# paramhanji/sin-inn

Measured on AMD Instinct MI355X. Metric: training frames/sec at 256x256 bs=16, higher is better.
Workload: dtype f32; 1 GPU; BASELINE configs[1]: 8-block INN (SRF, -c 4 x 2 levels), 256x256x3, fp32, synthetic clip (64 frames, lr_window 10), batch 16/GPU, full training step (fwd+bwd, rev+bwd, Adam); height=256, width=256, global_batch=16, num_coupling=4, architecture=SRF, parallelism=dp1, hip_graph=False

## Files before the change

### sin-inn_amd/csrc/conv_mfma.hip

```cpp
#include "conv_mfma_impl.h"

namespace sininn {

int conv_dispatch_k3(ConvDev& d, hipStream_t st, int force_cfg);
int conv_dispatch_k1(ConvDev& d, hipStream_t st, int force_cfg);
int conv32_dispatch_k3(ConvDev& d, hipStream_t st, int force_cfg, bool must);
int conv32_dispatch_k1(ConvDev& d, hipStream_t st, int force_cfg, bool must);
int wino_dispatch_k3(ConvDev& d, hipStream_t st, int cg2);

int g_conv_dma = 0;
static int g_force_cfg = 0;
static int g_force_ck = 0;
static int g_ablate = 0;

int conv_bf16_launch(const sininn_conv_args* a, hipStream_t st);
extern int g_bf16_force_ck16;

int conv_prepare(const sininn_conv_args* a, ConvDev& d) {
  SININN_CHECK(a != nullptr, "conv: null args");
  SININN_CHECK(a->ksize == 1 || a->ksize == 3, "conv: ksize %d not in {1,3}", a->ksize);
  SININN_CHECK(a->Cin > 0 && a->Cin % 8 == 0, "conv: Cin=%d must be a positive multiple of 8", a->Cin);
  SININN_CHECK(a->Np > 0 && a->Np % 16 == 0, "conv: Np=%d must be a positive multiple of 16", a->Np);
  SININN_CHECK(a->B > 0 && a->H > 0 && a->W > 0, "conv: bad image shape %dx%dx%d", a->B, a->H, a->W);
  SININN_CHECK((long)a->B * a->H * a->W * (long)(a->in_stride > a->out_stride ? a->in_stride : a->out_stride) < (1l << 31),
               "conv: tensor too large for 32-bit pixel offsets");
  SININN_CHECK(a->in && a->w && a->out, "conv: null tensor pointer");
  SININN_CHECK((a->in_stride >= a->Cin || a->in_group_stride > 0) && a->in_stride % 4 == 0 && aligned16(a->in),
               "conv: input must be 16-byte aligned with stride %% 4 == 0 (stride=%d)", a->in_stride);
  SININN_CHECK(aligned16(a->w), "conv: packed weights must be 16-byte aligned");
  const bool couple = a->mode == SININN_CONV_COUPLE_FWD || a->mode == SININN_CONV_COUPLE_INV;
  if (couple) {
    SININN_CHECK(a->Co > 0 && a->Co % 8 == 0 && a->Np == 2 * a->Co, "conv: coupling needs Np == 2*Co, Co %% 8 == 0 (Np=%d Co=%d)", a->Np, a->Co);
    SININN_CHECK(a->v != nullptr && a->v_stride >= a->Co, "conv: coupling needs v");
    SININN_CHECK(a->clamp > 0.f, "conv: clamp must be > 0");
    SININN_CHECK(a->out_stride >= a->Co, "conv: out_stride < Co");
  } else {
    SININN_CHECK(a->N > 0 && a->N <= a->Np && (a->out_stride >= a->N || a->out_group_stride > 0), "conv: bad N=%d (Np=%d, out_stride=%d)", a->N, a->Np, a->out_stride);
    if (a->mode == SININN_CONV_RELU) SININN_CHECK(a->bias != nullptr, "conv: RELU mode needs bias");
    if (a->mode == SININN_CONV_MASK) SININN_CHECK(a->mask != nullptr && (a->mask_stride >= a->N || a->mask_group_stride > 0), "conv: MASK mode needs mask");
    const bool cbwd = a->mode == SININN_CONV_ADD_CBWD_FWD || a->mode == SININN_CONV_ADD_CBWD_INV;
    if (a->mode == SININN_CONV_ADD || cbwd) SININN_CHECK(a->addend != nullptr, "conv: ADD mode needs addend");
    if (cbwd) SININN_CHECK(a->v && a->sbuf && a->out2 && a->Co == a->N && a->out_stride >= 2 * a->Co && a->clamp > 0.f, "conv: ADD_CBWD needs v, sbuf, out2, Co == N, out_stride >= 2*Co");
    if ((a->mode == SININN_CONV_LINEAR || a->mode == SININN_CONV_ADD) && a->mask)
      SININN_CHECK(a->Co >= 0 && a->Co % 4 == 0 && a->mask_stride >= a->N && a->mask_stride % 4 == 0 && aligned16(a->mask) && a->mask_group_stride <= 0,
                   "conv: LeakyReLU tail needs Co %% 4 == 0 and a 16-byte aligned pixel-major mask (Co=%d, mask_stride=%d)", a->Co, a->mask_stride);
    if (a->mode == SININN_CONV_IRN_FWD || a->mode == SININN_CONV_IRN_INV)
      SININN_CHECK(a->mask && a->v && a->mask_stride >= a->N && a->v_stride >= a->N && a->clamp > 0.f, "conv: IRN modes need aux (mask), v and clamp");
  }
  SININN_CHECK(aligned16(a->out) && a->out_stride % 4 == 0, "conv: out must be 16-byte aligned with stride %% 4 == 0");
  SININN_CHECK(!a->bias || aligned16(a->bias), "conv: bias must be 16-byte aligned");
  if (couple) {
    SININN_CHECK(aligned16(a->v) && a->v_stride % 4 == 0, "conv: v must be 16-byte aligned with stride %% 4 == 0");
    SININN_CHECK(!a->out2 || (aligned16(a->out2) && a->out2_stride % 4 == 0), "conv: out2 must be 16-byte aligned");
    SININN_CHECK(!a->sbuf || aligned16(a->sbuf), "conv: sbuf must be 16-byte aligned");
  }
  if (a->mode == SININN_CONV_MASK) SININN_CHECK(aligned16(a->mask) && a->mask_stride % 4 == 0, "conv: mask must be 16-byte aligned");
  SININN_CHECK(a->N % 4 == 0 || couple, "conv: N must be a multiple of 4");
  if ((a->mode == SININN_CONV_ADD || a->mode == SININN_CONV_ADD_CBWD_FWD || a->mode == SININN_CONV_ADD_CBWD_INV) && !a->addend_map)
    SININN_CHECK(aligned16(a->addend) && a->addend_stride % 4 == 0, "conv: addend must be 16-byte aligned");
  d.in = a->in; d.in_stride = a->in_stride; d.Cin = a->Cin;
  d.w = a->w; d.bias = a->bias; d.Np = a->Np;
  d.B = a->B; d.H = a->H; d.W = a->W;
  d.out = a->out; d.out_stride = a->out_stride; d.N = a->N; d.out_map = a->out_map;
  d.v = a->v; d.v_stride = a->v_stride; d.out2 = a->out2; d.out2_stride = a->out2_stride;
  d.sbuf = a->sbuf; d.logdet = a->logdet; d.Co = a->Co; d.clamp = a->clamp;
  d.mask = a->mask; d.mask_stride = a->mask_stride;
  d.addend = a->addend; d.addend_stride = a->addend_stride; d.addend_map = a->addend_map;
  d.mode = a->mode;
  d.col_tile = a->col_tile;
  d.stamp = a->stamp;
  d.ablate = g_ablate;
  d.in_chunk = a->in_group_stride > 0 ? a->in_group_stride : 8;
  d.out_gs = a->out_group_stride > 0 ? (size_t)a->out_group_stride : 0;
  d.mask_gs = a->mask_group_stride > 0 ? (size_t)a->mask_group_stride : 0;
  if (d.out_gs || d.mask_gs) {
    SININN_CHECK(a->winograd && (a->mode == SININN_CONV_RELU || a->mode == SININN_CONV_MASK) && a->N % 64 == 0 && a->N == a->Np,
                 "conv: channel-group-major out / mask needs a Winograd RELU / MASK conv with N == Np, N %% 64 == 0");
    SININN_CHECK(!d.mask_gs || a->mode == SININN_CONV_MASK, "conv: mask_group_stride without MASK mode");
  }
  if (a->in_group_stride > 0) SININN_CHECK(a->winograd && a->in_stride == 8, "conv: the channel-group-major input layout needs the Winograd kernels and in_stride == 8");
  if (a->winograd) {
    SININN_CHECK((unsigned long long)a->H * a->W * a->in_stride * 4ull < (1ull << 31),
                 "conv: one image of the input (%d x %d x stride %d floats) exceeds the 2 GB a Winograd block addresses", a->H, a->W, a->in_stride);
    SININN_CHECK((unsigned long long)(a->Cin / 8) * (unsigned long long)d.in_chunk * 4ull < (1ull << 32), "conv: input channel-group stride too large");
  }
  SININN_CHECK(a->mode >= 0 && a->mode <= SININN_CONV_ADD_CBWD_INV, "conv: unknown mode %d", a->mode);
  int ck = 8;
  for (int c : {32, 24, 16, 8}) if (a->Cin % c == 0) { ck = c; break; }
  if (g_force_ck && a->Cin % g_force_ck == 0 && g_force_ck % 8 == 0 && g_force_ck <= 32) ck = g_force_ck;
  d.CK = ck;
  d.tiles_x = d.tiles_y = 0;
  return 0;
}

int conv_launch(const sininn_conv_args* a, hipStream_t st) {
  SININN_CHECK(a != nullptr, "conv: null args");
  if (a->w_bf16) return conv_bf16_launch(a, st);
  ConvDev d;
  if (int rc = conv_prepare(a, d)) return rc;
  const bool couple = a->mode == SININN_CONV_COUPLE_FWD || a->mode == SININN_CONV_COUPLE_INV;
  if (a->winograd) {
    SININN_CHECK(a->ksize == 3, "conv: the Winograd pack needs ksize 3");
    d.col_tile = (couple && a->col_tile == 32) ? 32 : 16;
    if (couple && d.col_tile == 32) SININN_CHECK(a->Co % 16 == 0, "conv: col_tile 32 needs Co %% 16 == 0");
    return wino_dispatch_k3(d, st, g_force_cfg % 16);
  }
  const int tile = couple ? (a->col_tile == 32 ? 32 : 16) : ((a->Np % 32 == 0 && g_force_cfg < 10) ? 32 : 16);
  if (couple && tile == 32) SININN_CHECK(a->Co % 16 == 0, "conv: col_tile 32 needs Co %% 16 == 0 (Co=%d)", a->Co);
  const int fc = g_force_cfg % 10;
  if (tile == 32) {
    const int rc = (a->ksize == 3) ? conv32_dispatch_k3(d, st, fc, couple) : conv32_dispatch_k1(d, st, fc, couple);
    if (rc >= 0) return rc;
  }
  if (a->ksize == 3) return conv_dispatch_k3(d, st, fc);
  return conv_dispatch_k1(d, st, fc);
}

void conv_set_test_hooks(int force_cfg, int force_ck) {
  g_force_cfg = force_cfg % 100; g_force_ck = force_ck; g_ablate = force_cfg / 1000;
  g_bf16_force_ck16 = force_ck == 16;
  const int dma = (force_cfg / 100) % 10;
  if (dma) g_conv_dma = (dma == 1);
}

}
```

### sin-inn_amd/csrc/wino_impl.h

```cpp
#pragma once
#include "conv_mfma_impl.h"
#include "wino32_impl.h"

namespace sininn {

template <int NT, int HT, int CG>
__global__ __launch_bounds__(256 * CG, 2 / CG) void wino_kernel(ConvDev p) {
  constexpr int CK = 8;
  constexpr int NTHR = 256 * CG;
  constexpr int IW = 18, NPIX_IN = 18 * 18;
  constexpr int BG = NT * 16;
  constexpr int BN = CG * BG;
  constexpr int SI = 12, SU = 12;
  constexpr int PITCH = IW * SI + 4;
  constexpr int IN_F4 = (NPIX_IN * 2 + NTHR - 1) / NTHR;
  constexpr int U_F4 = (16 * BN * 2 + NTHR - 1) / NTHR;
  constexpr int IN_BUF = IW * PITCH + 4, U_BUF = 16 * BN * SU;
  constexpr bool U_EXACT = (16 * BN * 2) % NTHR == 0;

  extern __shared__ __attribute__((aligned(16))) float smem[];
  float* const in_lds0 = smem;
  float* const in_lds1 = smem + IN_BUF;
  float* const u_lds0 = smem + 2 * IN_BUF;
  float* const u_lds1 = u_lds0 + U_BUF;

  const int tid = threadIdx.x;
  stamp_begin(p);
  const int wave = (tid >> 6) & 3, grp = tid >> 8, lane = tid & 63;
  const int li = lane & 15, kq = lane >> 4;

  int bid = blockIdx.x;
  const int tx = bid % p.tiles_x; bid /= p.tiles_x;
  const int ty = bid % p.tiles_y;
  const int b = bid / p.tiles_y;
  const int y0 = ty * 16, x0 = tx * 16;
  const int n0 = blockIdx.y * BN;

  unsigned in_goff[IN_F4]; int in_loff[IN_F4];
#pragma unroll
  for (int r = 0; r < IN_F4; ++r) {
    const int f = tid + NTHR * r;
    const int pix = f >> 1, c4 = f & 1;
    const int py = pix / IW, px = pix - py * IW;
    const int gy = y0 + py - 1, gx = x0 + px - 1;
    const bool inside = pix < NPIX_IN;
    const bool inimg = inside && gy >= 0 && gy < p.H && gx >= 0 && gx < p.W;
    in_loff[r] = inside ? (py * PITCH + ((py >> 1) & 1) * 4 + px * SI + c4 * 4) : IW * PITCH;
    in_goff[r] = inimg ? (unsigned)(((gy * p.W + gx) * p.in_stride + c4 * 4) * 4) : BUF_OOB;
  }
  unsigned u_goff[U_F4]; int u_loff[U_F4];
#pragma unroll
  for (int r = 0; r < U_F4; ++r) {
    const int f = tid + NTHR * r;
    const int c4 = f & 1, col = (f >> 1) % BN, pos = (f >> 1) / BN;
    const bool inside = pos < 16;
    u_loff[r] = (U_EXACT || inside) ? ((pos * BN + col) * SU + c4 * 4) : -1;
    u_goff[r] = (inside && (n0 + col) < p.Np) ? (unsigned)(((pos * (p.Cin / CK) * p.Np + n0 + col) * CK + c4 * 4) * 4) : BUF_OOB;
  }
  const int nchunks = p.Cin / CK;

  const __amdgpu_buffer_rsrc_t in_rs = buf_rsrc(p.in + (size_t)b * p.H * p.W * p.in_stride), u_rs = buf_rsrc(p.w);
  const unsigned in_step = (unsigned)p.in_chunk * 4u, u_step = (unsigned)(p.Np * CK) * 4u;
  f32x4 in_reg[IN_F4], u_reg[U_F4];
  auto load_chunk = [&](int chunk) {
#pragma unroll
    for (int r = 0; r < IN_F4; ++r) in_reg[r] = buf_load4(in_rs, in_goff[r], (unsigned)chunk * in_step);
#pragma unroll
    for (int r = 0; r < U_F4; ++r) u_reg[r] = buf_load4(u_rs, u_goff[r], (unsigned)chunk * u_step);
  };
  auto store_chunk = [&](float* idst, float* udst) {
#pragma unroll
    for (int r = 0; r < IN_F4; ++r)
      *reinterpret_cast<f32x4*>(idst + in_loff[r]) = in_reg[r];
#pragma unroll
    for (int r = 0; r < U_F4; ++r)
      if (U_EXACT || u_loff[r] >= 0) *reinterpret_cast<f32x4*>(udst + u_loff[r]) = u_reg[r];
  };

  const int a_ty = 2 * wave + (li >> 3), a_tx = li & 7;
  const int a_base01 = (2 * a_ty) * PITCH + (a_ty & 1) * 4 + (2 * a_tx) * SI + 2 * kq;
  const int a_base23 = (2 * a_ty) * PITCH + ((a_ty + 1) & 1) * 4 + (2 * a_tx) * SI + 2 * kq;
  const int b_base = (grp * BG + li) * SU + 2 * kq;

  f32x4 acc[16][NT];
#pragma unroll
  for (int q = 0; q < 16; ++q)
#pragma unroll
    for (int n = 0; n < NT; ++n) acc[q][n] = (f32x4){0.f, 0.f, 0.f, 0.f};
  const bool tile1_live = (n0 + grp * BG + 16) < p.Np;

  load_chunk(0);
  store_chunk(in_lds0, u_lds0);
  if (nchunks > 1) load_chunk(1);
  __syncthreads();

  for (int it = 0; it < nchunks; ++it) {
    if (!(p.ablate & 1)) {
      if (it + 1 < nchunks) store_chunk(((it + 1) & 1) ? in_lds1 : in_lds0, ((it + 1) & 1) ? u_lds1 : u_lds0);
      if (it + 2 < nchunks) load_chunk(it + 2);
    }
    const unsigned A01 = lds_addr(((it & 1) ? in_lds1 : in_lds0) + a_base01);
    const unsigned A23 = lds_addr(((it & 1) ? in_lds1 : in_lds0) + a_base23);
    const unsigned Uc = lds_addr(((it & 1) ? u_lds1 : u_lds0) + b_base);

    f32x2 v[4][4];
    {
      f32x2 d[4][4];
      static_for<0, 16>([&](auto i) {
        constexpr int a = decltype(i)::value >> 2, c = decltype(i)::value & 3;
        d[a][c] = lds_read_b64<(a * PITCH + c * SI) * 4>(a < 2 ? A01 : A23);
      });
      asm volatile("s_waitcnt lgkmcnt(0)"
                   : "+v"(d[0][0]), "+v"(d[0][1]), "+v"(d[0][2]), "+v"(d[0][3]), "+v"(d[1][0]), "+v"(d[1][1]), "+v"(d[1][2]),
                     "+v"(d[1][3]), "+v"(d[2][0]), "+v"(d[2][1]), "+v"(d[2][2]), "+v"(d[2][3]), "+v"(d[3][0]), "+v"(d[3][1]),
                     "+v"(d[3][2]), "+v"(d[3][3]));
      f32x2 t[4][4];
#pragma unroll
      for (int c = 0; c < 4; ++c) {
        t[0][c] = d[0][c] - d[2][c];
        t[1][c] = d[1][c] + d[2][c];
        t[2][c] = d[2][c] - d[1][c];
        t[3][c] = d[1][c] - d[3][c];
      }
#pragma unroll
      for (int a = 0; a < 4; ++a) {
        v[a][0] = t[a][0] - t[a][2];
        v[a][1] = t[a][1] + t[a][2];
        v[a][2] = t[a][2] - t[a][1];
        v[a][3] = t[a][1] - t[a][3];
      }
    }
    constexpr int PF = 2;
    static_assert(NT == 2, "the wait counts below assume two column tiles per wave");
    f32x2 bf[PF + 1][NT];
    auto positions = [&](auto live1_tag) {
      constexpr bool LIVE1 = decltype(live1_tag)::value;
      static_for<0, PF>([&](auto qq) {
        constexpr int q = decltype(qq)::value;
        bf[q][0] = lds_read_b64<((q * BN) * SU) * 4>(Uc);
        if constexpr (LIVE1) bf[q][1] = lds_read_b64<((q * BN + 16) * SU) * 4>(Uc);
      });
      static_for<0, 16>([&](auto qq) {
        constexpr int q = decltype(qq)::value;
        if constexpr (q + PF < 16) {
          bf[(q + PF) % (PF + 1)][0] = lds_read_b64<(((q + PF) * BN) * SU) * 4>(Uc);
          if constexpr (LIVE1) bf[(q + PF) % (PF + 1)][1] = lds_read_b64<(((q + PF) * BN + 16) * SU) * 4>(Uc);
        }
        constexpr int newer = (q + PF < 16 ? PF : 15 - q) * (LIVE1 ? 2 : 1);
        if constexpr (LIVE1) lds_wait<newer>(bf[q % (PF + 1)][0], bf[q % (PF + 1)][1]);
        else lds_wait<newer>(bf[q % (PF + 1)][0]);
        acc[q][0] = __builtin_amdgcn_mfma_f32_16x16x4f32(v[q >> 2][q & 3].x, bf[q % (PF + 1)][0].x, acc[q][0], 0, 0, 0);
        if constexpr (LIVE1) acc[q][1] = __builtin_amdgcn_mfma_f32_16x16x4f32(v[q >> 2][q & 3].x, bf[q % (PF + 1)][1].x, acc[q][1], 0, 0, 0);
        acc[q][0] = __builtin_amdgcn_mfma_f32_16x16x4f32(v[q >> 2][q & 3].y, bf[q % (PF + 1)][0].y, acc[q][0], 0, 0, 0);
        if constexpr (LIVE1) acc[q][1] = __builtin_amdgcn_mfma_f32_16x16x4f32(v[q >> 2][q & 3].y, bf[q % (PF + 1)][1].y, acc[q][1], 0, 0, 0);
      });
    };
    if (tile1_live) positions(std::true_type{}); else positions(std::false_type{});
    if (!(p.ablate & 2)) __syncthreads();
  }

  {
    constexpr int TS = BN + 4;
    float* const T = smem;
#pragma unroll
    for (int n = 0; n < NT; ++n)
#pragma unroll
      for (int r = 0; r < 4; ++r) {
        float m[16];
#pragma unroll
        for (int q = 0; q < 16; ++q) m[q] = acc[q][n][r];
        float r0[4], r1[4];
#pragma unroll
        for (int c = 0; c < 4; ++c) {
          r0[c] = m[0 * 4 + c] + m[1 * 4 + c] + m[2 * 4 + c];
          r1[c] = m[1 * 4 + c] - m[2 * 4 + c] - m[3 * 4 + c];
        }
        const int tl = 4 * kq + r;
        const int oy = 2 * (2 * wave + (tl >> 3)), ox = 2 * (tl & 7);
        float* t00 = T + (oy * 16 + ox) * TS + grp * BG + n * 16 + li;
        t00[0] = r0[0] + r0[1] + r0[2];
        t00[TS] = r0[1] - r0[2] - r0[3];
        t00[16 * TS] = r1[0] + r1[1] + r1[2];
        t00[17 * TS] = r1[1] - r1[2] - r1[3];
      }
    __syncthreads();
    __shared__ float red[4 * CG];
    conv_epilogue_tile<16, BN, HT, NTHR>(p, T, b, y0, x0, n0, tid, red);
    stamp_end(p);
  }
}

template <int CG>
static int wino_launch(ConvDev& d, hipStream_t st) {
  constexpr int NT = 2, BN = CG * NT * 16;
  constexpr size_t lds_main = (size_t)(2 * (18 * (18 * 12 + 4) + 4) + 2 * 16 * BN * 12) * sizeof(float);
  constexpr size_t lds_epi = (size_t)256 * (BN + 4) * sizeof(float);
  constexpr size_t lds = lds_main > lds_epi ? lds_main : lds_epi;
  static_assert(lds <= 160 * 1024, "LDS tile too large");
  d.tiles_x = (d.W + 15) / 16;
  d.tiles_y = (d.H + 15) / 16;
  dim3 grid(d.tiles_x * d.tiles_y * d.B, (d.Np + BN - 1) / BN);
  auto k = (d.col_tile == 16) ? wino_kernel<NT, 8, CG> : wino_kernel<NT, 16, CG>;
  hipError_t e = hipFuncSetAttribute(reinterpret_cast<const void*>(k), hipFuncAttributeMaxDynamicSharedMemorySize, (int)lds);
  if (e != hipSuccess) { set_error("wino: cannot raise LDS limit to %zu", lds); return 1; }
  hipLaunchKernelGGL(k, grid, dim3(256 * CG), lds, st, d);
  SININN_LAUNCH_CHECK("wino");
  return 0;
}

static int wino_dispatch(ConvDev& d, hipStream_t st, int cg2 = 0) {
  const bool never32 = (cg2 & 4) != 0, always32 = (cg2 & 8) != 0;
  cg2 &= 3;
  const bool even_groups = ((d.Np + 31) / 32) % 2 == 0;
  bool wide = even_groups && d.Cin >= 64;
  if (cg2 == 1) wide = false;
  if (cg2 == 2) wide = even_groups;
  if (wide) return wino_launch<2>(d, st);
  const long blocks = (long)d.B * ((d.H + 15) / 16) * ((d.W + 15) / 16) * ((d.Np + 31) / 32);
  const bool use32 = d.col_tile == 16 && !never32 && (always32 || (d.Cin >= 128 && blocks <= 256));
  return use32 ? wino32_launch(d, st) : wino_launch<1>(d, st);
}

}
```

Measured before the change: 1960 frames/s.

## Add small-Cin Winograd kernel that stages input once and loops output groups

Adds a Winograd 3x3 conv kernel for Cin <= 40 and Np % 64 == 0. Each block loads its 18x18 input tile for all channel chunks into LDS once, then loops over every output-column group, double-buffering the transformed weights. The old path launched one block per output group and reloaded and re-transformed the input each time. This cuts redundant input traffic and launches fewer blocks, at the cost of lower parallelism (one block per spatial tile, 512 threads, occupancy 1) and more LDS. It is on by default and can be disabled with an env var or a test hook.

```diff
diff --git a/sin-inn_amd/csrc/conv_mfma.hip b/sin-inn_amd/csrc/conv_mfma.hip
--- a/sin-inn_amd/csrc/conv_mfma.hip
+++ b/sin-inn_amd/csrc/conv_mfma.hip
@@ -1,3 +1,4 @@
+#include <cstdlib>
 #include "conv_mfma_impl.h"
 
 namespace sininn {
@@ -11,6 +12,8 @@
 int g_conv_dma = 0;
 static int g_force_cfg = 0;
 static int g_force_ck = 0;
+static const bool g_smallk_env_off = getenv("SININN_WINO_SMALLK") != nullptr && atoi(getenv("SININN_WINO_SMALLK")) == 0;
+static bool g_smallk_hook_off = false;
 static int g_ablate = 0;
 
 int conv_bf16_launch(const sininn_conv_args* a, hipStream_t st);
@@ -103,7 +106,7 @@
     SININN_CHECK(a->ksize == 3, "conv: the Winograd pack needs ksize 3");
     d.col_tile = (couple && a->col_tile == 32) ? 32 : 16;
     if (couple && d.col_tile == 32) SININN_CHECK(a->Co % 16 == 0, "conv: col_tile 32 needs Co %% 16 == 0");
-    return wino_dispatch_k3(d, st, g_force_cfg % 16);
+    return wino_dispatch_k3(d, st, g_force_cfg % 16 + ((g_smallk_env_off || g_smallk_hook_off) ? 16 : 0));
   }
   const int tile = couple ? (a->col_tile == 32 ? 32 : 16) : ((a->Np % 32 == 0 && g_force_cfg < 10) ? 32 : 16);
   if (couple && tile == 32) SININN_CHECK(a->Co % 16 == 0, "conv: col_tile 32 needs Co %% 16 == 0 (Co=%d)", a->Co);
@@ -117,6 +120,7 @@
 }
 
 void conv_set_test_hooks(int force_cfg, int force_ck) {
+  g_smallk_hook_off = (force_ck & 64) != 0; force_ck &= ~64;
   g_force_cfg = force_cfg % 100; g_force_ck = force_ck; g_ablate = force_cfg / 1000;
   g_bf16_force_ck16 = force_ck == 16;
   const int dma = (force_cfg / 100) % 10;
diff --git a/sin-inn_amd/csrc/wino_impl.h b/sin-inn_amd/csrc/wino_impl.h
--- a/sin-inn_amd/csrc/wino_impl.h
+++ b/sin-inn_amd/csrc/wino_impl.h
@@ -1,6 +1,7 @@
 #pragma once
 #include "conv_mfma_impl.h"
 #include "wino32_impl.h"
+#include "wino_smallk_impl.h"
 
 namespace sininn {
 
@@ -209,6 +210,7 @@
 }
 
 static int wino_dispatch(ConvDev& d, hipStream_t st, int cg2 = 0) {
+  if (cg2 == 0 && wino_smallk_applies(d)) return wino_smallk_launch(d, st);
   const bool never32 = (cg2 & 4) != 0, always32 = (cg2 & 8) != 0;
   cg2 &= 3;
   const bool even_groups = ((d.Np + 31) / 32) % 2 == 0;
diff --git a/sin-inn_amd/csrc/wino_smallk_impl.h b/sin-inn_amd/csrc/wino_smallk_impl.h
--- /dev/null
+++ b/sin-inn_amd/csrc/wino_smallk_impl.h
@@ -0,0 +1,237 @@
+#pragma once
+#include "conv_mfma_impl.h"
+
+namespace sininn {
+
+template <int HT>
+__global__ __launch_bounds__(512, 1) void wino_smallk_kernel(ConvDev p) {
+  constexpr int CK = 8, NTHR = 512, NT = 2;
+  constexpr int IW = 18, NPIX_IN = 18 * 18;
+  constexpr int BG = 32, BN = 64;
+  constexpr int SI = 12, SU = 8;
+  constexpr int PITCH = IW * SI + 4;
+  constexpr int IN_F4 = (NPIX_IN * 2 + NTHR - 1) / NTHR;
+  constexpr int U_F4 = (16 * BN * 2) / NTHR;
+  constexpr int IN_BUF = IW * PITCH + 4, U_BUF = 16 * BN * SU;
+  constexpr int TS = BN + 4;
+  constexpr int T_SIZE = 256 * TS;
+  constexpr int UT_SIZE = T_SIZE > 2 * U_BUF ? T_SIZE : 2 * U_BUF;
+  constexpr int MAXCH = 5;
+  static_assert((16 * BN * 2) % NTHR == 0, "every thread slot of the U staging loop is a real quad");
+
+  extern __shared__ __attribute__((aligned(16))) float smem[];
+  float* const u_lds0 = smem;
+  float* const u_lds1 = smem + U_BUF;
+  float* const T = smem;
+  float* const in_lds = smem + UT_SIZE;
+  __shared__ float red[8];
+
+  const int tid = threadIdx.x;
+  stamp_begin(p);
+  const int wave = (tid >> 6) & 3, grp = tid >> 8, lane = tid & 63;
+  const int li = lane & 15, kq = lane >> 4;
+
+  int bid = blockIdx.x;
+  const int tx = bid % p.tiles_x; bid /= p.tiles_x;
+  const int ty = bid % p.tiles_y;
+  const int b = bid / p.tiles_y;
+  const int y0 = ty * 16, x0 = tx * 16;
+  const int nchunks = p.Cin / CK, ngroups = p.Np / BN;
+  const int nsteps = nchunks * ngroups;
+
+  const __amdgpu_buffer_rsrc_t in_rs = buf_rsrc(p.in + (size_t)b * p.H * p.W * p.in_stride), u_rs = buf_rsrc(p.w);
+  const unsigned in_step = (unsigned)p.in_chunk * 4u, u_step = (unsigned)(p.Np * CK) * 4u;
+
+  {
+    unsigned in_goff[IN_F4]; int in_loff[IN_F4];
+#pragma unroll
+    for (int r = 0; r < IN_F4; ++r) {
+      const int f = tid + NTHR * r;
+      const int pix = f >> 1, c4 = f & 1;
+      const int py = pix / IW, px = pix - py * IW;
+      const int gy = y0 + py - 1, gx = x0 + px - 1;
+      const bool inside = pix < NPIX_IN;
+      const bool inimg = inside && gy >= 0 && gy < p.H && gx >= 0 && gx < p.W;
+      in_loff[r] = inside ? (py * PITCH + ((py >> 1) & 1) * 4 + px * SI + c4 * 4) : IW * PITCH;
+      in_goff[r] = inimg ? (unsigned)(((gy * p.W + gx) * p.in_stride + c4 * 4) * 4) : BUF_OOB;
+    }
+    f32x4 in_reg[MAXCH][IN_F4];
+#pragma unroll
+    for (int ch = 0; ch < MAXCH; ++ch)
+      if (ch < nchunks) {
+#pragma unroll
+        for (int r = 0; r < IN_F4; ++r) in_reg[ch][r] = buf_load4(in_rs, in_goff[r], (unsigned)ch * in_step);
+      }
+#pragma unroll
+    for (int ch = 0; ch < MAXCH; ++ch)
+      if (ch < nchunks) {
+#pragma unroll
+        for (int r = 0; r < IN_F4; ++r) *reinterpret_cast<f32x4*>(in_lds + ch * IN_BUF + in_loff[r]) = in_reg[ch][r];
+      }
+  }
+
+  unsigned u_goff[U_F4]; int u_loff[U_F4];
+#pragma unroll
+  for (int r = 0; r < U_F4; ++r) {
+    const int f = tid + NTHR * r;
+    const int c4 = f & 1, col = (f >> 1) % BN, pos = (f >> 1) / BN;
+    u_loff[r] = (pos * BN + col) * SU + ((c4 ^ ((col >> 3) & 1)) * 4);
+    u_goff[r] = (unsigned)(((pos * nchunks * p.Np + col) * CK + c4 * 4) * 4);
+  }
+  f32x4 u_reg[U_F4];
+  auto load_u = [&](f32x4 (&dst)[U_F4], int g, int c) {
+    const unsigned off = (unsigned)c * u_step + (unsigned)(g * BN * CK) * 4u;
+#pragma unroll
+    for (int r = 0; r < U_F4; ++r) dst[r] = buf_load4(u_rs, u_goff[r], off);
+  };
+  auto store_u = [&](float* udst) {
+#pragma unroll
+    for (int r = 0; r < U_F4; ++r) *reinterpret_cast<f32x4*>(udst + u_loff[r]) = u_reg[r];
+  };
+
+  const int a_ty = 2 * wave + (li >> 3), a_tx = li & 7;
+  const int a_base01 = (2 * a_ty) * PITCH + (a_ty & 1) * 4 + (2 * a_tx) * SI + 2 * kq;
+  const int a_base23 = (2 * a_ty) * PITCH + ((a_ty + 1) & 1) * 4 + (2 * a_tx) * SI + 2 * kq;
+  const int b_base = (grp * BG + li) * SU + (((kq >> 1) ^ ((li >> 3) & 1)) * 4) + (kq & 1) * 2;
+
+  load_u(u_reg, 0, 0);
+  store_u(u_lds0);
+  if (nsteps > 1) { if (nchunks > 1) load_u(u_reg, 0, 1); else load_u(u_reg, 1, 0); }
+  __syncthreads();
+
+  for (int g = 0; g < ngroups; ++g) {
+    f32x4 acc[16][NT];
+#pragma unroll
+    for (int q = 0; q < 16; ++q)
+#pragma unroll
+      for (int n = 0; n < NT; ++n) acc[q][n] = (f32x4){0.f, 0.f, 0.f, 0.f};
+
+    for (int c = 0; c < nchunks; ++c) {
+      if (c + 1 < nchunks) {
+        store_u(((c + 1) & 1) ? u_lds1 : u_lds0);
+        if (c + 2 < nchunks) load_u(u_reg, g, c + 2);
+        else if (g + 1 < ngroups) load_u(u_reg, g + 1, 0);
+      }
+      const unsigned A01 = lds_addr(in_lds + c * IN_BUF + a_base01);
+      const unsigned A23 = lds_addr(in_lds + c * IN_BUF + a_base23);
+      const unsigned Uc = lds_addr(((c & 1) ? u_lds1 : u_lds0) + b_base);
+
+      f32x2 v[4][4];
+      {
+        f32x2 d[4][4];
+        static_for<0, 16>([&](auto i) {
+          constexpr int a = decltype(i)::value >> 2, cc = decltype(i)::value & 3;
+          d[a][cc] = lds_read_b64<(a * PITCH + cc * SI) * 4>(a < 2 ? A01 : A23);
+        });
+        asm volatile("s_waitcnt lgkmcnt(0)"
+                     : "+v"(d[0][0]), "+v"(d[0][1]), "+v"(d[0][2]), "+v"(d[0][3]), "+v"(d[1][0]), "+v"(d[1][1]), "+v"(d[1][2]),
+                       "+v"(d[1][3]), "+v"(d[2][0]), "+v"(d[2][1]), "+v"(d[2][2]), "+v"(d[2][3]), "+v"(d[3][0]), "+v"(d[3][1]),
+                       "+v"(d[3][2]), "+v"(d[3][3]));
+        f32x2 t[4][4];
+#pragma unroll
+        for (int cc = 0; cc < 4; ++cc) {
+          t[0][cc] = d[0][cc] - d[2][cc];
+          t[1][cc] = d[1][cc] + d[2][cc];
+          t[2][cc] = d[2][cc] - d[1][cc];
+          t[3][cc] = d[1][cc] - d[3][cc];
+        }
+#pragma unroll
+        for (int a = 0; a < 4; ++a) {
+          v[a][0] = t[a][0] - t[a][2];
+          v[a][1] = t[a][1] + t[a][2];
+          v[a][2] = t[a][2] - t[a][1];
+          v[a][3] = t[a][1] - t[a][3];
+        }
+      }
+      constexpr int PF = 2;
+      f32x2 bf[PF + 1][NT];
+      static_for<0, PF>([&](auto qq) {
+        constexpr int q = decltype(qq)::value;
+        bf[q][0] = lds_read_b64<((q * BN) * SU) * 4>(Uc);
+        bf[q][1] = lds_read_b64<((q * BN + 16) * SU) * 4>(Uc);
+      });
+      static_for<0, 16>([&](auto qq) {
+        constexpr int q = decltype(qq)::value;
+        if constexpr (q + PF < 16) {
+          bf[(q + PF) % (PF + 1)][0] = lds_read_b64<(((q + PF) * BN) * SU) * 4>(Uc);
+          bf[(q + PF) % (PF + 1)][1] = lds_read_b64<(((q + PF) * BN + 16) * SU) * 4>(Uc);
+        }
+        constexpr int newer = (q + PF < 16 ? PF : 15 - q) * 2;
+        lds_wait<newer>(bf[q % (PF + 1)][0], bf[q % (PF + 1)][1]);
+        acc[q][0] = __builtin_amdgcn_mfma_f32_16x16x4f32(v[q >> 2][q & 3].x, bf[q % (PF + 1)][0].x, acc[q][0], 0, 0, 0);
+        acc[q][1] = __builtin_amdgcn_mfma_f32_16x16x4f32(v[q >> 2][q & 3].x, bf[q % (PF + 1)][1].x, acc[q][1], 0, 0, 0);
+        acc[q][0] = __builtin_amdgcn_mfma_f32_16x16x4f32(v[q >> 2][q & 3].y, bf[q % (PF + 1)][0].y, acc[q][0], 0, 0, 0);
+        acc[q][1] = __builtin_amdgcn_mfma_f32_16x16x4f32(v[q >> 2][q & 3].y, bf[q % (PF + 1)][1].y, acc[q][1], 0, 0, 0);
+      });
+      __syncthreads();
+    }
+
+    const bool more = g + 1 < ngroups;
+    f32x4 u_nx[U_F4];
+#pragma unroll
+    for (int r = 0; r < U_F4; ++r) u_nx[r] = (f32x4){0.f, 0.f, 0.f, 0.f};
+    if (more && nchunks > 1) load_u(u_nx, g + 1, 1);
+
+    {
+      {
+#pragma unroll
+        for (int n = 0; n < NT; ++n)
+#pragma unroll
+          for (int r = 0; r < 4; ++r) {
+            float m[16];
+#pragma unroll
+            for (int q = 0; q < 16; ++q) m[q] = acc[q][n][r];
+            float r0[4], r1[4];
+#pragma unroll
+            for (int cc = 0; cc < 4; ++cc) {
+              r0[cc] = m[0 * 4 + cc] + m[1 * 4 + cc] + m[2 * 4 + cc];
+              r1[cc] = m[1 * 4 + cc] - m[2 * 4 + cc] - m[3 * 4 + cc];
+            }
+            const int tl = 4 * kq + r;
+            const int oy = 2 * (2 * wave + (tl >> 3)), ox = 2 * (tl & 7);
+            float* t00 = T + (oy * 16 + ox) * TS + grp * BG + n * 16 + li;
+            t00[0] = r0[0] + r0[1] + r0[2];
+            t00[TS] = r0[1] - r0[2] - r0[3];
+            t00[16 * TS] = r1[0] + r1[1] + r1[2];
+            t00[17 * TS] = r1[1] - r1[2] - r1[3];
+          }
+      }
+      __syncthreads();
+      int tid_e = tid;
+      asm volatile("" : "+v"(tid_e));
+      conv_epilogue_tile<16, BN, HT, NTHR>(p, T, b, y0, x0, g * BN, tid_e, red);
+    }
+
+    if (more) {
+      __syncthreads();
+      store_u(u_lds0);
+      if (nchunks > 1) {
+#pragma unroll
+        for (int r = 0; r < U_F4; ++r) u_reg[r] = u_nx[r];
+      } else if (g + 2 < ngroups) {
+        load_u(u_reg, g + 2, 0);
+      }
+      __syncthreads();
+    }
+  }
+  stamp_end(p);
+}
+
+static bool wino_smallk_applies(const ConvDev& d) { return d.Cin <= 40 && d.Cin % 8 == 0 && d.Np % 64 == 0; }
+
+static int wino_smallk_launch(ConvDev& d, hipStream_t st) {
+  constexpr size_t in_buf = (size_t)(18 * (18 * 12 + 4) + 4), u_pair = (size_t)2 * 16 * 64 * 8, t_tile = (size_t)256 * 68;
+  const size_t lds = ((size_t)(d.Cin / 8) * in_buf + (t_tile > u_pair ? t_tile : u_pair)) * sizeof(float);
+  if (lds > 160 * 1024 - 64) { set_error("wino small-K: LDS tile too large (%zu)", lds); return 1; }
+  d.tiles_x = (d.W + 15) / 16;
+  d.tiles_y = (d.H + 15) / 16;
+  dim3 grid(d.tiles_x * d.tiles_y * d.B);
+  auto k = (d.col_tile == 16) ? wino_smallk_kernel<8> : wino_smallk_kernel<16>;
+  hipError_t e = hipFuncSetAttribute(reinterpret_cast<const void*>(k), hipFuncAttributeMaxDynamicSharedMemorySize, (int)lds);
+  if (e != hipSuccess) { set_error("wino small-K: cannot raise LDS limit to %zu", lds); return 1; }
+  hipLaunchKernelGGL(k, grid, dim3(512), lds, st, d);
+  SININN_LAUNCH_CHECK("wino small-K");
+  return 0;
+}
+
+}
```

Result: no change. 1968 frames/s, median of 6 (+0.4%).
